# kausaltech/reina-model

Measured on NVIDIA B200. Metric: agent-days/sec (HUS 1.7M), higher is better.
Workload: dtype int32/f32 state, f64 uniforms

## Files before the change

### reina_b200/csrc/engine.cu

```cuda
#include "state.cuh"
#include "boundary.cuh"
#include "sweep.cuh"
#include "contacts.cuh"
#include "shard.cuh"
#include "setup.cuh"
#include "run.cuh"

static thread_local char g_err[512];
#define CK(call) do { cudaError_t e_ = (call); if (e_ != cudaSuccess) { snprintf(g_err, sizeof g_err, "%s:%d %s: %s", __FILE__, __LINE__, #call, cudaGetErrorString(e_)); return 1; } } while (0)

#define MAX_GROUPS 8
struct ReplicaGroup {
    int r0, R;
    int sweep_blocks, list_blocks, resolve_blocks;
    cudaStream_t stream;
    cudaEvent_t ev_stagger, ev_join;
    cudaGraphExec_t graph[2];
};

struct rb_engine {
    rb_config cfg;
    Eng G;
    cudaStream_t stream;
    cudaEvent_t ev0, ev1;
// ... 47 lines not shown
static int load_nccl() {
    if (g_nccl.dl) return 0;
    void *h = dlopen("libnccl.so.2", RTLD_NOW | RTLD_NOLOAD | RTLD_GLOBAL);
    if (!h) h = dlopen("libnccl.so.2", RTLD_NOW | RTLD_GLOBAL);
    if (!h) h = dlopen("libnccl.so", RTLD_NOW | RTLD_GLOBAL);
    if (!h) { snprintf(g_err, sizeof g_err, "cannot load libnccl.so.2: %s", dlerror()); return 1; }
    g_nccl.GetUniqueId = (ncclResult_t(*)(ncclUniqueId *))dlsym(h, "ncclGetUniqueId");
    g_nccl.CommInitRank = (ncclResult_t(*)(ncclComm_t *, int, ncclUniqueId, int))dlsym(h, "ncclCommInitRank");
    g_nccl.AllGather = (ncclResult_t(*)(const void *, void *, size_t, ncclDataType_t, ncclComm_t, cudaStream_t))dlsym(h, "ncclAllGather");
    g_nccl.AllReduce = (ncclResult_t(*)(const void *, void *, size_t, ncclDataType_t, ncclRedOp_t, ncclComm_t, cudaStream_t))dlsym(h, "ncclAllReduce");
    g_nccl.CommDestroy = (ncclResult_t(*)(ncclComm_t))dlsym(h, "ncclCommDestroy");
    g_nccl.GetErrorString = (const char *(*)(ncclResult_t))dlsym(h, "ncclGetErrorString");
    if (!g_nccl.GetUniqueId || !g_nccl.CommInitRank || !g_nccl.AllGather || !g_nccl.AllReduce || !g_nccl.CommDestroy || !g_nccl.GetErrorString) {
        snprintf(g_err, sizeof g_err, "libnccl.so.2 lacks a required symbol"); return 1;
    }
    g_nccl.dl = h;
    return 0;
}
#define NK(call) do { ncclResult_t r_ = (call); if (r_ != ncclSuccess) { snprintf(g_err, sizeof g_err, "%s:%d %s: %s", __FILE__, __LINE__, #call, g_nccl.GetErrorString(r_)); return 1; } } while (0)


template <typename T> static int dalloc(rb_engine *e, T **p, size_t n) {
    void *q = nullptr;
    cudaError_t err = cudaMalloc(&q, n * sizeof(T));
    if (err != cudaSuccess) { snprintf(g_err, sizeof g_err, "cudaMalloc(%zu bytes): %s", n * sizeof(T), cudaGetErrorString(err)); return 1; }
    e->allocs.push_back(q);
    *p = (T *)q;
    return 0;
}
static uint32_t pow2_at_least(uint64_t x) { uint32_t p = 1024; while (p < x) p <<= 1; return p; }

extern "C" const char *rb_last_error(void) { return g_err; }

static int init_population(rb_engine *e, uint32_t seed, bool sparse) {
    const Eng &G = e->G;
    k_init_counters<<<G.R, 128, 0, e->stream>>>(G, seed, e->cfg.hospital_beds, e->cfg.icu_units);
    if (sparse) k_init<true><<<dim3(e->sweep_blocks, G.R), 256, 0, e->stream>>>(G);
    else k_init<false><<<dim3(e->sweep_blocks, G.R), 256, 0, e->stream>>>(G);
    k_init_bitmaps<<<dim3(8, G.R), 256, 0, e->stream>>>(G);
    k_clear_lists<<<128, 256, 0, e->stream>>>(G);
    e->launches += 4;
    CK(cudaGetLastError());
    return 0;
}

static int setup_groups(rb_engine *e, int sms);
static void group_config(int R, int *n_groups, int *wave_pct);

static int resolve_grid(int n_agents, int sms, int pct, int replicas) {
    long long b = ((long long)n_agents / 128 + 255) / 256;
    long long cap = (long long)sms * 16 * pct / 100 / replicas; if (cap < 64) cap = 64;
    if (const char *s = getenv("RB_RESOLVE_BLOCKS")) cap = b = atoi(s);
    if (b > cap) b = cap;
    return b < 1 ? 1 : (int)b;
}

extern "C" void rb_destroy(rb_engine *e) {
    if (!e) return;
    cudaSetDevice(e->cfg.device);
    cudaStreamSynchronize(e->stream);
    if (e->have_graphs) {
        if (e->n_groups <= 1) { cudaGraphExecDestroy(e->graph[0]); cudaGraphExecDestroy(e->graph[1]); }
        else for (int g = 0; g < e->n_groups; g++) { cudaGraphExecDestroy(e->grp[g].graph[0]); cudaGraphExecDestroy(e->grp[g].graph[1]); }
    }
    for (int g = 0; g < e->n_groups && e->n_groups > 1; g++) {
        cudaStreamDestroy(e->grp[g].stream); cudaEventDestroy(e->grp[g].ev_stagger); cudaEventDestroy(e->grp[g].ev_join);
    }
    if (e->n_groups > 1) cudaEventDestroy(e->ev_fork);
    if (e->have_sh_graphs) { cudaGraphExecDestroy(e->sh_graph[0]); cudaGraphExecDestroy(e->sh_graph[1]); }
    for (int k = 0; k < e->n_peer_open; k++) if (k != e->G.rank && e->G.xpeer[k]) cudaIpcCloseMemHandle(e->G.xpeer[k]);
    if (e->comm) g_nccl.CommDestroy(e->comm);
    for (void *p : e->allocs) cudaFree(p);
    if (e->h_stage) { cudaFreeHost(e->h_stage); for (int i = 0; i < 4; i++) cudaEventDestroy(e->ev_stage[i]); }
    cudaEventDestroy(e->ev0); cudaEventDestroy(e->ev1);
    cudaStreamDestroy(e->stream);
    delete e;
}

extern "C" int rb_create(const rb_config *cfg, const int32_t *age_counts, const int32_t *group_of_age,
                         const rb_variant *variants, const int32_t *import_lo, const int32_t *import_hi,
                         const float *import_cum, rb_engine **out) {
    if (cfg->n_ages > RB_MAX_AGES || cfg->n_variants > RB_MAX_VARIANTS || cfg->n_import_classes > RB_MAX_IMPORT_CLASSES ||
        cfg->n_groups > 16 || cfg->n_replicas < 1 || cfg->n_agents < 1) {
        snprintf(g_err, sizeof g_err, "config exceeds compiled limits"); return 1;
    }
    int ndev = 0;
    if (cudaGetDeviceCount(&ndev) != cudaSuccess || ndev == 0) {
        snprintf(g_err, sizeof g_err, "no CUDA device: reina_b200 has no CPU fallback"); return 2;
    }
    CK(cudaSetDevice(cfg->device));
    if (const char *s = getenv("RB_L2_FETCH")) cudaDeviceSetLimit(cudaLimitMaxL2FetchGranularity, (size_t)atoi(s));
    rb_engine *e = new rb_engine();
    e->cfg = *cfg; e->day = 0; e->last_ms = 0; e->launches = 0; e->h2d_bytes = 0; e->d2h_bytes = 0; e->have_graphs = false; e->comm = nullptr; e->comm_rank = 0; e->comm_size = 1; e->sharded = false; e->merge_blocks = 1;
    e->has_ipc = false; e->h_stage = nullptr; e->n_stage = 0; e->n_groups = 1; e->wide_ctas = 1; e->n_peer_open = 0; e->launch_err = cudaSuccess; e->shard_timing = getenv("RB_SHARD_TIMING") != nullptr;
    e->xepoch = 0; e->d_xepoch = nullptr; e->have_sh_graphs = false;
    { int lo = 0, hi = 0; CK(cudaDeviceGetStreamPriorityRange(&lo, &hi)); e->prio_high = hi; e->prio = (cfg->n_replicas >= 32 && cfg->n_replicas < 128) ? 1 : 0; if (const char *s = getenv("RB_PRIO")) e->prio = atoi(s); }
    CK(cudaStreamCreateWithFlags(&e->stream, cudaStreamNonBlocking));
    CK(cudaEventCreate(&e->ev0)); CK(cudaEventCreate(&e->ev1));
    Eng &G = e->G;
    memset(&G, 0, sizeof G);
    const int N = cfg->n_agents, R = cfg->n_replicas;
    G.N = N; G.Npad = (N + 3) & ~3; G.n_ages = cfg->n_ages; G.n_groups = cfg->n_groups; G.n_variants = cfg->n_variants;
    G.R = R; G.max_days = cfg->max_days; G.row_len = RB_N_ATTRS * cfg->n_groups + RB_N_SCALARS;
    G.n_import_classes = cfg->n_import_classes;
    G.rank = 0; G.nranks = 1;
    int bits = 1; while ((1u << bits) < (uint32_t)N) bits++;
    G.fhalf = (bits + 1) / 2;
    e->age_start.resize(cfg->n_ages + 1);
    int64_t tot = 0;
    for (int a = 0; a < cfg->n_ages; a++) { e->age_start[a] = (int32_t)tot; tot += age_counts[a]; }
    e->age_start[cfg->n_ages] = (int32_t)tot;
    if (tot != N) { snprintf(g_err, sizeof g_err, "age_counts sum %lld != n_agents %d", (long long)tot, N); delete e; return 1; }
    for (int i = 0; i < cfg->n_import_classes; i++) {
        const float w = import_cum[i] - (i ? import_cum[i - 1] : 0.0f);
        if (import_lo[i] < 0 || import_hi[i] >= cfg->n_ages || import_lo[i] > import_hi[i]) { snprintf(g_err, sizeof g_err, "import class %d: bad age band", i); delete e; return 1; }
        if ((w > 0.0f || i == cfg->n_import_classes - 1) && e->age_start[import_hi[i] + 1] - e->age_start[import_lo[i]] <= 0) {
            snprintf(g_err, sizeof g_err, "import class %d (ages %d-%d) can be drawn but is empty", i, import_lo[i], import_hi[i]); delete e; return 1;
        }
    }
    float cc = cfg->contact_capacity > 0 ? cfg->contact_capacity : 1.0f;
    G.cap_items = pow2_at_least((uint64_t)((double)N * cc) + 4096);
    G.cap_succ = pow2_at_least((uint64_t)N / 8 + 4096);
    G.cap_events = pow2_at_least((uint64_t)N / 16 + 2048);
    G.cap_queue = pow2_at_least((uint64_t)N / 8 + 2048);
    const size_t RN = (size_t)R * G.Npad;
    cudaDeviceProp prop; CK(cudaGetDeviceProperties(&prop, cfg->device));
    const int sms = prop.multiProcessorCount;
    e->run_ctas = 0; e->run_boundary_ctas = 1;
    {
        int per_sm = 0;
        CK(cudaOccupancyMaxActiveBlocksPerMultiprocessor(&per_sm, k_run, RUN_THREADS, 0));
        const long long total = (long long)per_sm * sms;
        bool on = false;
        if (const char *s = getenv("RB_PERSISTENT")) on = atoi(s) != 0;
        if (on && total >= 2LL * R) {
            long long t = total / R; if (t > 64) t = 64;
            if (const char *s = getenv("RB_RUN_CTAS")) { const int v = atoi(s); if (v >= 1 && (long long)v * R <= total) t = v; }
            e->run_ctas = (int)t;
            int b = 1; while (b * 2 <= t && b * 2 <= 16) b *= 2;
            e->run_boundary_ctas = b;
        }
    }
    {
        int ng, pct;
        group_config(R, &ng, &pct);
        long long ctas = (long long)sms * SW_CTAS_PER_SM * (ng > 1 ? pct : 100) / 100 / ((R + ng - 1) / ng);
        if (ctas < 1) ctas = 1;
        long long S = 2 * ctas * SW_WARPS, most = (long long)N / 256;
        if (e->run_ctas) S = 2LL * e->run_ctas * RUN_WARPS;
        if (S > most) S = most;
        G.n_seg = (uint32_t)(S < 1 ? 1 : S);
        G.seg_cap = ((uint32_t)N + G.n_seg - 1) / G.n_seg;
    }
    G.sus_words = ((G.Npad + 31) / 32 + 32 + 3) & ~3;
    if (dalloc(e, &G.hot, RN) || dalloc(e, &G.perm, RN) || dalloc(e, &G.rec, RN) ||
        dalloc(e, &G.sus, (size_t)R * G.sus_words) || dalloc(e, &G.det, (size_t)R * G.sus_words) || dalloc(e, &G.alist, (size_t)R * 2 * G.n_seg * G.seg_cap) || dalloc(e, &G.seg_n, (size_t)R * 2 * G.n_seg) || dalloc(e, &G.items, (size_t)R * G.cap_items) || dalloc(e, &G.succ, (size_t)R * G.cap_succ) ||
        dalloc(e, &G.ev_key, (size_t)R * G.cap_events) || dalloc(e, &G.ev_agent, (size_t)R * G.cap_events) ||
        dalloc(e, &G.q_key, (size_t)R * 2 * G.cap_queue) || dalloc(e, &G.q_agent, (size_t)R * 2 * G.cap_queue) ||
        dalloc(e, &G.ctr, (size_t)R) || dalloc(e, &G.stats, (size_t)R * (cfg->max_days + 1) * G.row_len) ||
        dalloc(e, &e->d_sched, (size_t)cfg->max_days + 1) ||
        dalloc(e, &e->d_moments, 2 * ((size_t)cfg->max_days + 1) * G.row_len + 2)) { rb_destroy(e); return 1; }
    G.sched = e->d_sched;
    e->h_sched.assign(cfg->max_days + 1, rb_day_params());
    e->n_table_slots = 1024;
    if (dalloc(e, &e->d_tables, (size_t)e->n_table_slots)) { rb_destroy(e); return 1; }
    CK(cudaMemset(e->d_tables, 0, sizeof(DevTable *) * e->n_table_slots));
    G.tables = e->d_tables;
    e->tables.assign(e->n_table_slots, nullptr);
    rb_variant *dv; int32_t *d_as, *d_ga, *d_ilo, *d_ihi; float *d_icum; uint8_t *d_ab;
    if (dalloc(e, &dv, (size_t)cfg->n_variants) || dalloc(e, &d_as, (size_t)cfg->n_ages + 1) || dalloc(e, &d_ga, (size_t)cfg->n_ages) ||
        dalloc(e, &d_ilo, (size_t)RB_MAX_IMPORT_CLASSES) || dalloc(e, &d_ihi, (size_t)RB_MAX_IMPORT_CLASSES) ||
        dalloc(e, &d_icum, (size_t)RB_MAX_IMPORT_CLASSES) || dalloc(e, &d_ab, (size_t)(G.Npad >> 10) + 2)) { rb_destroy(e); return 1; }
    {
        std::vector<uint8_t> ab((size_t)(G.Npad >> 10) + 2);
        int age = 0;
        for (size_t b = 0; b < ab.size(); b++) {
            int64_t a = (int64_t)b << 10; if (a > N - 1) a = N - 1;
            while (age < cfg->n_ages - 1 && e->age_start[age + 1] <= a) age++;
            ab[b] = (uint8_t)age;
        }
        CK(cudaMemcpy(d_ab, ab.data(), ab.size(), cudaMemcpyHostToDevice));
    }
    e->h_variants.assign(variants, variants + cfg->n_variants);
    CK(cudaMemcpy(dv, variants, sizeof(rb_variant) * cfg->n_variants, cudaMemcpyHostToDevice));
    CK(cudaMemcpy(d_as, e->age_start.data(), sizeof(int32_t) * (cfg->n_ages + 1), cudaMemcpyHostToDevice));
    CK(cudaMemcpy(d_ga, group_of_age, sizeof(int32_t) * cfg->n_ages, cudaMemcpyHostToDevice));
    CK(cudaMemcpy(d_ilo, import_lo, sizeof(int32_t) * cfg->n_import_classes, cudaMemcpyHostToDevice));
    CK(cudaMemcpy(d_ihi, import_hi, sizeof(int32_t) * cfg->n_import_classes, cudaMemcpyHostToDevice));
    CK(cudaMemcpy(d_icum, import_cum, sizeof(float) * cfg->n_import_classes, cudaMemcpyHostToDevice));
    G.age_blk = d_ab; G.variants = dv; G.age_start = d_as; G.group_of_age = d_ga; G.import_lo = d_ilo; G.import_hi = d_ihi; G.import_cum = d_icum;
    e->age_counts.assign(age_counts, age_counts + cfg->n_ages);
    CK(cudaMemset(G.stats, 0, sizeof(int32_t) * (size_t)R * (cfg->max_days + 1) * G.row_len));
    CK(cudaMemset(e->d_sched, 0, sizeof(rb_day_params) * ((size_t)cfg->max_days + 1)));
    int want = ((int)G.n_seg + SW_WARPS - 1) / SW_WARPS;
    int per_rep = sms * SW_CTAS_PER_SM / R; if (per_rep < 1) per_rep = 1;
    e->sweep_blocks = want < per_rep ? want : per_rep; if (e->sweep_blocks < 1) e->sweep_blocks = 1;
    e->list_blocks = sms * EX_CTAS_PER_SM / R; if (e->list_blocks < 2) e->list_blocks = 2;
    e->resolve_blocks = resolve_grid(G.N, sms, 100, R);
    if (init_population(e, cfg->seed, false)) { rb_destroy(e); return 1; }
    CK(cudaStreamSynchronize(e->stream));
    if (e->run_ctas) e->n_groups = 1;
    else if (setup_groups(e, sms)) { rb_destroy(e); return 1; }
    e->wide_ctas = 1;
    G.wide_min = 2048;
    if (e->n_groups == 1 && R * 4 <= sms && N >= 4000000) { e->wide_ctas = 16; while (e->wide_ctas * R > sms) e->wide_ctas >>= 1; }
    if (const char *s = getenv("RB_WIDE_CTAS")) { int v = atoi(s); if (v >= 1 && v <= WIDE_MAX_CTAS && v * R <= sms) e->wide_ctas = v; }
    if (const char *s = getenv("RB_WIDE_MIN")) G.wide_min = atoi(s);
    if (const char *s = getenv("RB_WIDE_CTAS")) {
        const int v = atoi(s); int b = 1; while (b * 2 <= v && b * 2 <= e->run_ctas) b *= 2;
        if (e->run_ctas) e->run_boundary_ctas = b;
    }
    *out = e;
    return 0;
}

static void group_config(int R, int *n_groups, int *wave_pct) {
    int ng = R >= 32 ? 4 : 1, pct = R >= 32 ? 50 : 100;
    if (const char *s = getenv("RB_GROUPS")) ng = atoi(s);
    if (const char *s = getenv("RB_GROUP_WAVE_PCT")) pct = atoi(s);
    if (pct < 1) pct = 100;
    if (ng > MAX_GROUPS) ng = MAX_GROUPS;
    if (ng > R) ng = R;
    if (ng < 1) ng = 1;
    *n_groups = ng; *wave_pct = pct;
}
static int setup_groups(rb_engine *e, int sms) {
    const int R = e->G.R;
    int ng, pct;
    group_config(R, &ng, &pct);
    e->n_groups = ng;
    if (ng == 1) return 0;
    CK(cudaEventCreateWithFlags(&e->ev_fork, cudaEventDisableTiming));
    const Eng &G = e->G;
    const int want = ((int)G.n_seg + SW_WARPS - 1) / SW_WARPS;
    for (int g = 0; g < ng; g++) {
        ReplicaGroup &q = e->grp[g];
        q.r0 = (int)((long long)R * g / ng); q.R = (int)((long long)R * (g + 1) / ng) - q.r0;
        int per = sms * SW_CTAS_PER_SM * pct / 100 / q.R; if (per < 1) per = 1;
        q.sweep_blocks = want < per ? want : per;
        q.list_blocks = sms * EX_CTAS_PER_SM * pct / 100 / q.R; if (q.list_blocks < 2) q.list_blocks = 2;
        q.resolve_blocks = resolve_grid(G.N, sms, pct, q.R);
        CK(cudaStreamCreateWithFlags(&q.stream, cudaStreamNonBlocking));
        CK(cudaEventCreateWithFlags(&q.ev_stagger, cudaEventDisableTiming));
        CK(cudaEventCreateWithFlags(&q.ev_join, cudaEventDisableTiming));
    }
    return 0;
}

__global__ void k_set_word(uint32_t *p, uint32_t v) { *p = v; }
static void bump_xepoch(rb_engine *e) {
    e->xepoch++;
    if (e->d_xepoch) { k_set_word<<<1, 1, 0, e->stream>>>(e->d_xepoch, e->xepoch); e->launches++; }
}

extern "C" int rb_reset(rb_engine *e, uint32_t seed) {
    CK(cudaSetDevice(e->cfg.device));
    CK(cudaStreamSynchronize(e->stream));
    e->cfg.seed = seed;
    e->day = 0;
    bump_xepoch(e);
    if (init_population(e, seed, true)) return 1;
    if (e->has_ipc) {
        k_initial_state<<<e->G.R, 32, 0, e->stream>>>(e->G, e->ipc);
        k_rebuild_lists<<<dim3(e->sweep_blocks, e->G.R), 256, 0, e->stream>>>(e->G);
        e->launches += 2;
    }
    CK(cudaGetLastError());
    return 0;
}

extern "C" int rb_set_initial_state(rb_engine *e, const int32_t *ipc7) {
    CK(cudaSetDevice(e->cfg.device));
    if (e->day != 0 || e->has_ipc) { snprintf(g_err, sizeof g_err, "rb_set_initial_state: once, before the first step"); return 1; }
    for (int i = 0; i < 7; i++) if (ipc7[i] < 0) { snprintf(g_err, sizeof g_err, "rb_set_initial_state: negative count"); return 1; }
    e->ipc.dead = ipc7[0]; e->ipc.in_icu = ipc7[1]; e->ipc.in_ward = ipc7[2]; e->ipc.confirmed = ipc7[3];
    e->ipc.incubating = ipc7[4]; e->ipc.ill = ipc7[5]; e->ipc.recovered = ipc7[6];
    e->has_ipc = true;
    k_initial_state<<<e->G.R, 32, 0, e->stream>>>(e->G, e->ipc);
    k_rebuild_lists<<<dim3(e->sweep_blocks, e->G.R), 256, 0, e->stream>>>(e->G);
    e->launches += 2;
    CK(cudaGetLastError());
    CK(cudaStreamSynchronize(e->stream));
    return 0;
}

#define TABLE_HOST_BYTES (offsetof(DevTable, guide))
static int stage_slot(rb_engine *e, DevTable **h, int *slot) {
    if (!e->h_stage) {
        CK(cudaMallocHost((void **)&e->h_stage, TABLE_HOST_BYTES * 4));
        for (int i = 0; i < 4; i++) CK(cudaEventCreateWithFlags(&e->ev_stage[i], cudaEventDisableTiming));
        e->n_stage = 0;
    }
    const int k = e->n_stage & 3;
    if (e->n_stage >= 4) CK(cudaEventSynchronize(e->ev_stage[k]));
    e->n_stage++;
    *h = (DevTable *)((uint8_t *)e->h_stage + TABLE_HOST_BYTES * k); *slot = k;
    return 0;
}

extern "C" int rb_set_contact_table(rb_engine *e, int32_t epoch, const int32_t *n_rows, const double *cum_p,
                                    const int32_t *age_lo, const int32_t *age_hi, const uint8_t *place,
                                    const float *mask_p, const double *nr_contacts, const double *ncontact_cdf) {
    if (epoch < 0 || epoch >= e->n_table_slots) { snprintf(g_err, sizeof g_err, "table epoch out of range"); return 1; }
    CK(cudaSetDevice(e->cfg.device));
    for (int age = 0; age < e->cfg.n_ages; age++) {
        if (n_rows[age] < 0 || n_rows[age] > RB_MAX_ROWS) { snprintf(g_err, sizeof g_err, "contact table: n_rows[%d] = %d", age, n_rows[age]); return 1; }
        if (e->age_counts[age] == 0) continue;
        for (int i = 0; i < n_rows[age]; i++) {
            const int k = age * RB_MAX_ROWS + i;
// ... 804 lines not shown
```

### reina_b200/csrc/state.cuh

```cuda
#ifndef REINA_B200_STATE_CUH
#define REINA_B200_STATE_CUH

#include <cuda_runtime.h>
#include <stdint.h>
#include <stdio.h>
#include <string.h>

#include <dlfcn.h>
#include <nccl.h>

#include <algorithm>
#include <vector>

#include "../../include/reina_b200.h"
#include "rng.cuh"

#define MAX_INFECTEES 64
#define MAX_CONTACTS 128

#define H_STATE(h) ((h) & 7u)
#define H_SEV(h) (((h) >> 3) & 7u)
#define H_DET (1u << 6)
#define H_QUEUED (1u << 7)
#define H_VAR(h) (((h) >> 8) & 3u)
#define H_FRESH (1u << 10)
#define H_INCL (1u << 11)
#define H_LIST (1u << 12)
#define H_VACC (1u << 13)
#define H_DL(h) (((h) >> 14) & 255u)
#define H_DOI(h) (((h) >> 22) & 31u)
#define H_PEND (1u << 27)
#define H_DAYS_MASK ((255u << 14) | (31u << 22))
#define H_SET_STATE(h, s) (((h) & ~7u) | (uint32_t)(s))
#define H_SET_DL(h, d) (((h) & ~(255u << 14)) | ((uint32_t)(d) << 14))
#define H_SET_DOI(h, d) (((h) & ~(31u << 22)) | ((uint32_t)(d) << 22))

#define KEY_IDLE 0xFFFFFFFFFFFFFFFFull
#define QKEY_SWEEP (1ull << 62)
#define CT_DEAD (1ull << 61)
#define CT_DECIDED (1ull << 60)
#define CT_KEYMASK ((1ull << 60) - 1ull)

enum { EV_HOSP_CLAIM = 0, EV_WARD_RELEASE = 1, EV_TO_ICU = 2, EV_ICU_RELEASE = 3 };

#define MAX_RANKS 16
#define WIDE_MAX_CTAS 64
#define SORT_SMEM 2048
#ifndef PRE_THREADS
#define PRE_THREADS 512
#endif
#define NEG_INF (-(1 << 29))

#ifndef GUIDE_BITS
#define GUIDE_BITS 12
#endif
struct DevTable {
    int32_t n_rows[RB_MAX_AGES];
    float nr_contacts[RB_MAX_AGES];
    double ncdf[RB_MAX_AGES][2][RB_NCDF];
    double cum_p[RB_MAX_AGES][RB_MAX_ROWS];
    uint32_t cum24[RB_MAX_AGES][RB_MAX_ROWS];
    int32_t start[RB_MAX_AGES][RB_MAX_ROWS];
    int32_t size[RB_MAX_AGES][RB_MAX_ROWS];
    float mask_p[RB_MAX_AGES][RB_MAX_ROWS];
    uint8_t place[RB_MAX_AGES][RB_MAX_ROWS];
    uint8_t lo_age[RB_MAX_AGES][RB_MAX_ROWS], hi_age[RB_MAX_AGES][RB_MAX_ROWS];
    uint8_t susc_uniform[RB_MAX_AGES][RB_MAX_ROWS];
    uint8_t nguide[RB_MAX_AGES][2][256];
    uint32_t guide[RB_MAX_AGES][1 << GUIDE_BITS];
};

struct Attempt { uint32_t cand, parent; unsigned long long key; };

struct __align__(32) AgentRec {
    unsigned long long winner;
    int32_t infector, first_child, next_sib;
    uint32_t inf_key;
    uint32_t cold;
    int16_t vacc_day, pad;
};

struct RepCtr {
    int32_t counts[RB_N_ATTRS][RB_MAX_AGES];
    alignas(128) int32_t beds;
    int32_t icu, avail_beds, avail_icu;
    int32_t problem, epoch, testing_mode, day;
    float p_detected_anyway, p_successful_tracing;
    uint32_t seed, start;
    uint32_t fkey[4];
    uint32_t n_queue, qsel;
    uint32_t n_queue_prev;
    uint32_t any_vacc;
    uint32_t lsel;
    uint32_t ct_ever;
    uint32_t n_q_base;
    uint32_t drained;
    int32_t ct_cases;
    int32_t vacc_cursor[RB_MAX_VACC];
    alignas(128) uint32_t n_items;
    alignas(128) uint32_t n_succ;
    alignas(128) int32_t exposed_per_day;
    int32_t total_infectors, total_infections;
    alignas(128) uint32_t n_events;
    uint32_t n_newq;
    uint32_t n_upd;
    alignas(128) int32_t daily_contacts[RB_N_PLACES];
    int32_t by_variant[RB_MAX_VARIANTS];
    alignas(128) int32_t drain_det[RB_MAX_AGES];
    alignas(128) uint32_t n_l0;
    uint32_t n_l1, n_edges;
    alignas(128) unsigned int run_bar;
    unsigned int run_exit;
    alignas(128) unsigned int wide_bar;
    alignas(128) uint32_t wide_day;
    int32_t wide_mp[WIDE_MAX_CTAS][4];
    long long dbg_t[16];
    long long dbg_last;
};

struct Eng {
    int32_t dbg;
    int32_t N, Npad, n_ages, n_groups, n_variants, R, max_days, row_len, n_import_classes, fhalf;
    uint32_t cap_items, cap_succ, cap_events, cap_queue;
    uint32_t *hot;
    uint32_t *perm;
    AgentRec *rec;
    uint32_t *sus;
    int32_t sus_words;
    uint32_t *det;
    uint2 *alist;
    uint2 *seg_n;
    uint32_t n_seg, seg_cap;
    uint2 *items;
    Attempt *succ;
    unsigned long long *ev_key; int32_t *ev_agent;
    unsigned long long *q_key; int32_t *q_agent;
    RepCtr *ctr;
    int32_t *stats;
    const rb_day_params *sched;
    DevTable *const *tables;
    const rb_variant *variants;
    const int32_t *age_start;
    const uint8_t *age_blk;
    const int32_t *group_of_age;
    const int32_t *import_lo, *import_hi; const float *import_cum;
    int32_t rank, nranks;
    int32_t wide_min;
    int32_t r0;
    uint8_t *xbuf; size_t xslot;
    uint8_t *xpeer[MAX_RANKS];
    int32_t xp2p; const uint32_t *xepoch;
    uint32_t xcap_q, xcap_ev, xcap_upd, xcap_succ;
};

#define XFLAG_BYTES 256
#define SH_SHIFT 12
__device__ __forceinline__ uint32_t xflag_value(const Eng &G, int day) { return *G.xepoch * 65536u + (uint32_t)day + 1u; }
__device__ __forceinline__ bool owns(const Eng &G, uint32_t a) { return G.nranks == 1 || (int)((a >> SH_SHIFT) % (uint32_t)G.nranks) == G.rank; }

struct XSlot {
    RepCtr *hdr;
    unsigned long long *q_key; int32_t *q_agent;
    unsigned long long *ev_key; int32_t *ev_agent;
    uint2 *upd;
    struct Attempt *succ;
};
__host__ __device__ inline size_t xalign(size_t x) { return (x + 255) & ~(size_t)255; }
__host__ __device__ inline size_t xslot_bytes(uint32_t cq, uint32_t ce, uint32_t cu, uint32_t cs) {
    return xalign(sizeof(RepCtr)) + xalign(8ull * cq) + xalign(4ull * cq) + xalign(8ull * ce) + xalign(4ull * ce) + xalign(8ull * cu) + xalign(16ull * cs);
}
__device__ __forceinline__ XSlot xslot_of(const Eng &G, int rk, int day) {
    uint8_t *p = G.xp2p ? G.xpeer[rk] + XFLAG_BYTES + (size_t)(day & 1) * G.xslot : G.xbuf + (size_t)rk * G.xslot;
    XSlot s;
    s.hdr = (RepCtr *)p; p += xalign(sizeof(RepCtr));
    s.q_key = (unsigned long long *)p; p += xalign(8ull * G.xcap_q);
    s.q_agent = (int32_t *)p; p += xalign(4ull * G.xcap_q);
    s.ev_key = (unsigned long long *)p; p += xalign(8ull * G.xcap_ev);
    s.ev_agent = (int32_t *)p; p += xalign(4ull * G.xcap_ev);
    s.upd = (uint2 *)p; p += xalign(8ull * G.xcap_upd);
    s.succ = (struct Attempt *)p;
    return s;
}

__device__ __forceinline__ int age_of(const Eng &G, int32_t a) {
    int age = __ldg(&G.age_blk[a >> 10]);
    while (a >= __ldg(&G.age_start[age + 1])) age++;
    return age;
}
__device__ __forceinline__ int age_in_band(const Eng &G, int32_t a, int lo, int hi) {
    hi += 1;
    while (hi - lo > 1) { int mid = (lo + hi) >> 1; if (__ldg(&G.age_start[mid]) <= a) lo = mid; else hi = mid; }
    return lo;
}
__device__ __forceinline__ uint32_t sweep_slot(const Eng &G, const RepCtr *c, uint32_t a) {
    return feistel(a, (uint32_t)G.N, G.fhalf, c->fkey[0], c->fkey[1], c->fkey[2], c->fkey[3]);
}
__device__ __forceinline__ uint32_t sweep_pos(const Eng &G, int r, const RepCtr *c, uint32_t a) {
    const uint32_t s = G.perm[(size_t)r * G.Npad + a];
    return s >= c->start ? s - c->start : s + (uint32_t)G.N - c->start;
}
__device__ __forceinline__ void mark_detected(const Eng &G, int r, int32_t a) {
    atomicOr(&G.det[(size_t)r * G.sus_words + (a >> 5)], 1u << (a & 31));
}
__device__ __forceinline__ void count_add(RepCtr *c, int attr, int age, int d) { atomicAdd(&c->counts[attr][age], d); }
__device__ __forceinline__ void set_problem(RepCtr *c, int p) { atomicCAS(&c->problem, 0, p); }

__device__ __forceinline__ int symptom_severity(const rb_variant *v, int age, float val, bool vacc_eff) {
    float vmod = 1.0f;
    if (vacc_eff) vmod = vmod * 0.1f;
    float syc = v->tab[RB_T_SYMPTOMATIC][age];
    if (val >= syc) return RB_ASYMPTOMATIC;
    syc = syc * vmod;
    float dohc = v->tab[RB_T_DEATH_OUTSIDE_HOSPITAL][age];
    if (dohc != 0.0f) {
        if (val < dohc * syc) return RB_FATAL;
        val = (val - dohc) / (1.0f - dohc);
    }
    float sc = v->tab[RB_T_SEVERE][age], cc = v->tab[RB_T_CRITICAL][age], fc = v->tab[RB_T_FATAL][age];
    if (val < ((fc * cc) * sc) * syc) return RB_FATAL;
    if (val < (cc * sc) * syc) return RB_CRITICAL;
    if (val < sc * syc) return RB_SEVERE;
    return RB_MILD;
}

__device__ __forceinline__ uint2 *seg_ptr(const Eng &G, int r, uint32_t which, uint32_t s) {
    return G.alist + (((size_t)r * 2 + which) * G.n_seg + s) * G.seg_cap;
}
__device__ __forceinline__ uint2 *seg_count(const Eng &G, int r, uint32_t which, uint32_t s) {
    return G.seg_n + ((size_t)r * 2 + which) * G.n_seg + s;
}
__device__ __forceinline__ void list_add(const Eng &G, int r, RepCtr *c, uint32_t which, uint32_t a, uint32_t w) {
    const uint32_t s = a % G.n_seg;
    const uint32_t k = atomicAdd(&seg_count(G, r, which, s)->y, 1u);
    if (k < G.seg_cap) seg_ptr(G, r, which, s)[G.seg_cap - 1u - k] = make_uint2(a, w); else set_problem(c, RB_OTHER_FAILURE);
}

__device__ void device_infect(const Eng &G, int r, RepCtr *c, int32_t t, int32_t src, uint32_t src_h, int variant,
                              int slot, bool fresh, int list, bool has_list) {
    const size_t base = (size_t)r * G.Npad;
    const int day = c->day;
    uint32_t old = 0; int32_t prev_child = -1;
    if (src >= 0) {
        old = atomicAdd(&G.rec[base + src].cold, 1u);
        prev_child = atomicExch(&G.rec[base + src].first_child, t);
    }
    const int vd = c->any_vacc ? (int)G.rec[base + t].vacc_day : -1;
    const int age = age_of(G, t);
    const rb_variant *v0 = &G.variants[0];
    const bool vacc_eff = vd >= 0 && (day - vd) > 14;
    int sev = 0, dl = 0;
    if (owns(G, (uint32_t)t)) {
        u32x4 x = philox(c->seed, (uint32_t)t, (uint32_t)day, PU_SEVERITY, 0);
        sev = symptom_severity(v0, age, u01f(x.x), vacc_eff);
        dl = clamp255(round_to_int(gamma_f(c->seed, (uint32_t)t, (uint32_t)day, PU_INCUB, v0->incubation_kappa, v0->incubation_theta)));
    }
    if (src >= 0) {
        variant = (int)H_VAR(src_h);
        G.rec[base + t].infector = src;
        if ((src_h & H_LIST) && (old & 0xffffu) >= MAX_INFECTEES) set_problem(c, RB_TOO_MANY_INFECTEES);
        G.rec[base + t].inf_key = ((uint32_t)day << 8) | (uint32_t)slot;
        G.rec[base + t].next_sib = prev_child;
    }
    uint32_t nh = (vd >= 0 ? H_VACC : 0u) | RB_INCUBATION | ((uint32_t)sev << 3) | ((uint32_t)variant << 8) | ((uint32_t)dl << 14);
    if (fresh) nh |= H_FRESH;
    if (has_list) nh |= H_LIST;
    G.hot[base + t] = nh;
    G.perm[base + t] = sweep_slot(G, c, (uint32_t)t);
    atomicAnd(&G.sus[(size_t)r * G.sus_words + (t >> 5)], ~(1u << (t & 31)));
    if (list >= 0 && owns(G, (uint32_t)t)) list_add(G, r, c, (uint32_t)list, (uint32_t)t, nh);
    count_add(c, RB_A_SUSCEPTIBLE, age, -1);
    count_add(c, RB_A_INFECTED, age, 1);
    count_add(c, RB_A_ALL_INFECTED, age, 1);
    count_add(c, RB_A_NEW_INFECTIONS, age, 1);
    {
        const unsigned act = __activemask();
        const unsigned grp = __match_any_sync(act, variant);
        if ((int)(threadIdx.x & 31) == __ffs(grp) - 1) atomicAdd(&c->by_variant[variant], __popc(grp));
    }
}

#endif
```

### reina_b200/csrc/sweep.cuh

```cuda
#ifndef REINA_B200_SWEEP_CUH
#define REINA_B200_SWEEP_CUH
#include "state.cuh"

#ifndef SW_THREADS
#define SW_THREADS 128
#endif
#define SW_WARPS (SW_THREADS / 32)
#define SW_RCAP 64
#ifndef SW_CTAS_PER_SM
#define SW_CTAS_PER_SM 9
#endif

struct WarpRings {
    uint32_t ea[SW_RCAP], ed[SW_RCAP];
    uint32_t ta[SW_RCAP], tw[SW_RCAP];
};

__device__ __forceinline__ uint32_t ring_push(uint32_t *ra, uint32_t *rb, uint32_t tail, bool want, uint32_t x, uint32_t y, int lane) {
    const uint32_t m = __ballot_sync(0xffffffffu, want);
    if (want) { uint32_t p = (tail + __popc(m & ((1u << lane) - 1u))) & (SW_RCAP - 1); ra[p] = x; rb[p] = y; }
    return tail + __popc(m);
}

__device__ __forceinline__ void seg_append(const Eng &G, RepCtr *c, uint2 *out, uint32_t &out_n, bool want, uint32_t a, uint32_t w, int lane) {
    const uint32_t m = __ballot_sync(0xffffffffu, want);
    if (want) {
        const uint32_t p = out_n + __popc(m & ((1u << lane) - 1u));
        if (p < G.seg_cap) out[p] = make_uint2(a, w); else set_problem(c, RB_OTHER_FAILURE);
    }
    out_n += __popc(m);
}

struct SweepOut {
    RepCtr *cd;
    unsigned long long *q_key; int32_t *q_agent; uint32_t cap_q;
    unsigned long long *ev_key; int32_t *ev_agent; uint32_t cap_ev;
    uint2 *upd; uint32_t cap_upd;
};
__device__ __forceinline__ SweepOut sweep_out(const Eng &G, int r, RepCtr *c) {
    SweepOut O;
    if (!G.xbuf) {
        const size_t qb = ((size_t)r * 2 + (c->qsel ^ 1u)) * G.cap_queue;
        O.cd = c; O.q_key = G.q_key + qb; O.q_agent = G.q_agent + qb; O.cap_q = G.cap_queue;
        O.ev_key = G.ev_key + (size_t)r * G.cap_events; O.ev_agent = G.ev_agent + (size_t)r * G.cap_events; O.cap_ev = G.cap_events;
        O.upd = nullptr; O.cap_upd = 0;
    } else {
        const XSlot x = xslot_of(G, G.rank, c->day);
        O.cd = x.hdr; O.q_key = x.q_key; O.q_agent = x.q_agent; O.cap_q = G.xcap_q;
        O.ev_key = x.ev_key; O.ev_agent = x.ev_agent; O.cap_ev = G.xcap_ev; O.upd = x.upd; O.cap_upd = G.xcap_upd;
    }
    return O;
}

__device__ __forceinline__ void stage_expose(const Eng &G, int r, RepCtr *c, RepCtr *cd, const DevTable *tb, const WarpRings &W, uint32_t head, uint32_t m,
                                             uint2 *items, int lane) {
    uint32_t ncont = 0, desc = 0, a = 0;
    if ((uint32_t)lane < m) {
        a = W.ea[(head + lane) & (SW_RCAP - 1)];
        desc = W.ed[(head + lane) & (SW_RCAP - 1)];
        bool detected = false;
        if (c->ct_ever) detected = (__ldg(&G.det[(size_t)r * G.sus_words + (a >> 5)]) >> (a & 31)) & 1u;
        if (!detected) {
            const int age = age_of(G, (int32_t)a);
            const int cls = (desc >> 22) & 1u;
            u32x4 x = philox(c->seed, a, (uint32_t)c->day, PU_NCONTACT, 0);
            const double u = u01d(x.x, x.y);
            const double *cdf = tb->ncdf[age][cls];
            const int limit = cls ? 5 : 100;
            const uint32_t ng = tb->nguide[age][cls][x.x >> 24];
            int k = (int)(ng & 127u);
            if (ng & 128u) while (k < limit && !(u < __ldg(&cdf[k]))) k++;
            ncont = (uint32_t)k;
            desc = (desc & ~(1u << 22)) | ((uint32_t)age << 7);
        }
    }
    const uint32_t cnt = (ncont + 3u) >> 2;
    uint32_t incl = cnt | (ncont << 16);
#pragma unroll
    for (int o = 1; o < 32; o <<= 1) { uint32_t t = __shfl_up_sync(0xffffffffu, incl, o); if (lane >= o) incl += t; }
    const uint32_t tot = __shfl_sync(0xffffffffu, incl, 31), wtot = tot & 0xffffu;
    if (wtot == 0) return;
    uint32_t gbase = 0;
    if (lane == 31) { gbase = atomicAdd(&c->n_items, wtot); atomicAdd(&cd->exposed_per_day, (int)(tot >> 16)); }
    gbase = __shfl_sync(0xffffffffu, gbase, 31);
    if (gbase + wtot > G.cap_items) { if (lane == 0) set_problem(cd, RB_OTHER_FAILURE); return; }
    uint2 *mine = items + gbase + ((incl & 0xffffu) - cnt);
    for (uint32_t g = 0; g < cnt; g++) {
        const uint32_t left = ncont - 4u * g;
        mine[g] = make_uint2(a, desc | g | (((left < 4u ? left : 4u) - 1u) << 5));
    }
}

__device__ __forceinline__ void emit_event(const Eng &G, int r, const SweepOut &O, RepCtr *c, int32_t a, int type) {
    uint32_t idx = atomicAdd(&O.cd->n_events, 1u);
    if (idx < O.cap_ev) {
        O.ev_key[idx] = ((unsigned long long)sweep_pos(G, r, c, (uint32_t)a) << 2) | (unsigned)type;
        O.ev_agent[idx] = a;
    } else set_problem(O.cd, RB_OTHER_FAILURE);
}

__device__ __forceinline__ uint32_t transition(const Eng &G, int r, RepCtr *c, const SweepOut &O, int32_t a, uint32_t h, uint32_t &lw) {
    RepCtr *cd = O.cd;
    const size_t base = (size_t)r * G.Npad;
    const int day = c->day;
    const int age = age_of(G, a);
    const uint32_t st = H_STATE(h), sev = H_SEV(h);
    const rb_variant *v = &G.variants[H_VAR(h)];
    uint32_t extra = 0;
    if (st == RB_INCUBATION) {
        float T = (sev == RB_FATAL)
            ? gamma_f(c->seed, (uint32_t)a, (uint32_t)day, PU_ONSET, v->onset_death_kappa, v->onset_death_theta)
            : gamma_f(c->seed, (uint32_t)a, (uint32_t)day, PU_ONSET, v->onset_recovery_kappa, v->onset_recovery_theta);
        float f = T;
        if (sev != RB_ASYMPTOMATIC && sev != RB_MILD) f = f * v->ratio_before_hospitalisation;
        const uint32_t dl = (uint32_t)clamp255(round_to_int(f));
        float w = 0.0f, u = 0.0f;
        if (sev == RB_SEVERE) w = T * (1.0f - v->ratio_before_hospitalisation);
        else if (sev == RB_CRITICAL || sev == RB_FATAL) {
            w = T * v->ratio_in_ward;
            u = ((1.0f - v->ratio_in_ward) - v->ratio_before_hospitalisation) * T;
        }
        const uint32_t wd = (uint32_t)clamp255(round_to_int(w)), ud = (uint32_t)clamp255(round_to_int(u));
        if (wd | ud) atomicOr(&G.rec[base + a].cold, (wd << 16) | (ud << 24));
        h = H_SET_DL(H_SET_STATE(h, RB_ILLNESS), dl);
        if (sev != RB_ASYMPTOMATIC && !(h & H_DET)) {
            bool q = false;
            const int mode = c->testing_mode;
            if (mode == RB_ALL_WITH_SYMPTOMS || mode == RB_ALL_WITH_SYMPTOMS_CT) q = true;
            else if (mode == RB_ONLY_SEVERE_SYMPTOMS) {
                if (sev >= RB_SEVERE) q = true;
                else {
                    u32x4 x = philox(c->seed, (uint32_t)a, (uint32_t)day, PU_SEEK, 0);
                    q = chance(u01d(x.x, x.y), c->p_detected_anyway);
                }
            }
            if (q && !(h & H_QUEUED)) {
                h |= H_QUEUED;
                uint32_t idx = atomicAdd(&cd->n_newq, 1u);
                if (idx < O.cap_q) {
                    O.q_key[idx] = QKEY_SWEEP | sweep_pos(G, r, c, (uint32_t)a);
                    O.q_agent[idx] = a;
                } else set_problem(cd, RB_OTHER_FAILURE);
            }
        }
        if (h & H_QUEUED) extra = H_DET;
    } else if (st == RB_ILLNESS) {
        if (sev == RB_FATAL) {
            h = H_SET_STATE(h, RB_DEAD) & ~H_LIST;
            count_add(cd, RB_A_INFECTED, age, -1); count_add(cd, RB_A_DEAD, age, 1); count_add(cd, RB_A_NON_HOSPITAL_DEATHS, age, 1);
        } else if (sev >= RB_SEVERE) {
            if (!(h & H_DET)) { h |= H_DET; count_add(cd, RB_A_DETECTED, age, 1); count_add(cd, RB_A_ALL_DETECTED, age, 1); }
            emit_event(G, r, O, c, a, EV_HOSP_CLAIM);
            extra = H_PEND;
        } else {
            h = H_SET_STATE(h, RB_RECOVERED) & ~H_LIST;
            count_add(cd, RB_A_INFECTED, age, -1); count_add(cd, RB_A_RECOVERED, age, 1);
        }
    } else {
        int type;
        if (st == RB_HOSPITALIZED && (sev == RB_CRITICAL || sev == RB_FATAL)) { type = EV_TO_ICU; extra = H_PEND; }
        else {
            type = st == RB_IN_ICU ? EV_ICU_RELEASE : EV_WARD_RELEASE;
            count_add(cd, st == RB_IN_ICU ? RB_A_IN_ICU : RB_A_IN_WARD, age, -1);
            count_add(cd, RB_A_INFECTED, age, -1);
            if (sev == RB_FATAL) { h = H_SET_STATE(h, RB_DEAD) & ~H_LIST; count_add(cd, RB_A_DEAD, age, 1); count_add(cd, RB_A_NON_HOSPITAL_DEATHS, age, 1); }
            else { h = H_SET_STATE(h, RB_RECOVERED) & ~H_LIST; count_add(cd, RB_A_RECOVERED, age, 1); }
        }
        emit_event(G, r, O, c, a, type);
    }
    lw = h | extra;
    return h;
}

__device__ __forceinline__ void stage_slow(const Eng &G, int r, RepCtr *c, RepCtr *cd, const WarpRings &W, uint32_t head, uint32_t m,
                                           uint32_t next, int lane) {
    const SweepOut O = sweep_out(G, r, c);
    const size_t base = (size_t)r * G.Npad;
    const bool on = (uint32_t)lane < m;
    bool keep = false, changed = false, removed = false;
    int infected_others = 0;
    uint32_t a = 0, lw = 0, h = 0;
    if (on) {
        a = W.ta[(head + lane) & (SW_RCAP - 1)];
        const uint32_t w = W.tw[(head + lane) & (SW_RCAP - 1)];
        const uint32_t hot = G.hot[base + a];
        if (w & H_PEND) {
            h = hot & ~H_FRESH;
            if (H_STATE(h) < RB_RECOVERED) { uint32_t dl = H_DL(h); if (dl > 0) dl--; h = H_SET_DL(h, dl); }
        } else h = (hot & ~(H_DAYS_MASK | H_FRESH)) | (w & H_DAYS_MASK);
        const uint32_t st = H_STATE(h);
        if (st >= RB_RECOVERED) {
            removed = true;
            infected_others = (int)(G.rec[base + a].cold & 0xffffu);
            G.hot[base + a] = hot | H_INCL;
        } else if (H_DL(h) == 0) {
            h = transition(G, r, c, O, (int32_t)a, h, lw);
            G.hot[base + a] = h;
            keep = true; changed = true;
        } else { lw = h; keep = true; }
    }
    const uint32_t rm = __ballot_sync(0xffffffffu, removed);
    if (rm) {
#pragma unroll
        for (int o = 16; o > 0; o >>= 1) infected_others += __shfl_xor_sync(0xffffffffu, infected_others, o);
        if (lane == 0) { atomicAdd(&cd->total_infectors, __popc(rm)); if (infected_others) atomicAdd(&cd->total_infections, infected_others); }
    }
    if (keep) list_add(G, r, cd, next, a, lw);
    if (O.upd) {
        const uint32_t mk = __ballot_sync(0xffffffffu, changed);
        uint32_t b = 0;
        if (lane == 0 && mk) b = atomicAdd(&O.cd->n_upd, (uint32_t)__popc(mk));
        b = __shfl_sync(0xffffffffu, b, 0);
        if (changed) {
            const uint32_t idx = b + __popc(mk & ((1u << lane) - 1u));
            if (idx < O.cap_upd) O.upd[idx] = make_uint2(a, h); else set_problem(O.cd, RB_OTHER_FAILURE);
        }
    }
}

__device__ __forceinline__ void stage_entry(const Eng &G, uint32_t &w, bool &keep, bool &want_e, bool &want_t, uint32_t &desc) {
    const uint32_t st = H_STATE(w);
    if ((w & H_PEND) || st >= RB_RECOVERED) { want_t = true; return; }
    if (w & H_FRESH) { w &= ~H_FRESH; keep = true; return; }
    const uint32_t sev = H_SEV(w), var = H_VAR(w);
    uint32_t dl = H_DL(w);
    if (st == RB_INCUBATION || st == RB_ILLNESS) {
        const int dayidx = st == RB_INCUBATION ? -(int)dl : (int)H_DOI(w);
        if (!(w & H_DET) && dayidx >= -10 && dayidx <= 10 && G.variants[var].iot[dayidx + 10] != 0.0f) {
            want_e = true;
            const uint32_t cls = (st == RB_ILLNESS && sev != RB_ASYMPTOMATIC) ? 1u : 0u;
            desc = ((uint32_t)(dayidx + 10) << 14) | ((sev == RB_ASYMPTOMATIC ? 1u : 0u) << 19) | (var << 20) | (cls << 22);
        }
        if (st == RB_ILLNESS) { uint32_t doi = H_DOI(w); if (doi < 31) doi++; w = H_SET_DOI(w, doi); }
    }
    if (dl > 0) dl--;
    w = H_SET_DL(w, dl);
    if (dl == 0) want_t = true; else keep = true;
}

__device__ __forceinline__ void sweep_warp(const Eng &G, const int r, const uint32_t first, const uint32_t n_warps, WarpRings &W, const int lane) {
    RepCtr *c = &G.ctr[r];
    const DevTable *tb = G.tables[c->epoch];
    uint2 *items = G.items + (size_t)r * G.cap_items;
    RepCtr *cd = !G.xbuf ? c : xslot_of(G, G.rank, c->day).hdr;
    const uint32_t cur = c->lsel;
    uint32_t e_head = 0, e_tail = 0, t_head = 0, t_tail = 0;

    uint2 cnt_next = make_uint2(0u, 0u);
    if (first < G.n_seg) cnt_next = *seg_count(G, r, cur, first);
    for (uint32_t seg = first; ; seg += n_warps) {
        const bool tail = seg >= G.n_seg;
        const uint2 cnt = cnt_next;
        cnt_next = make_uint2(0u, 0u);
        if (seg + n_warps < G.n_seg) cnt_next = *seg_count(G, r, cur, seg + n_warps);
        const uint32_t nf = min(cnt.x, G.seg_cap), n = min(cnt.x + cnt.y, G.seg_cap);
        const uint2 *in = seg_ptr(G, r, cur, tail ? 0u : seg);
        uint2 *out = seg_ptr(G, r, cur ^ 1u, tail ? 0u : seg);
        uint32_t out_n = 0;
        const uint32_t gap = G.seg_cap - n;
        auto entry = [&](uint32_t i) { return __ldcs(&in[i < nf ? i : i + gap]); };
        uint2 ent = make_uint2(0u, 0u);
        if ((uint32_t)lane < n) ent = entry(lane);
        uint32_t i0 = 0;
        bool again;
        do {
            if (i0 < n) {
                const bool valid = i0 + lane < n;
                const uint2 cur_ent = ent;
                if (i0 + 32 + lane < n) ent = entry(i0 + 32 + lane);
                bool keep = false, want_e = false, want_t = false;
                uint32_t w = cur_ent.y, desc = 0;
                if (valid) stage_entry(G, w, keep, want_e, want_t, desc);
                seg_append(G, cd, out, out_n, keep, cur_ent.x, w, lane);
                e_tail = ring_push(W.ea, W.ed, e_tail, want_e, cur_ent.x, desc, lane);
                t_tail = ring_push(W.ta, W.tw, t_tail, want_t, cur_ent.x, w, lane);
                __syncwarp();
            }
            const uint32_t e_av = e_tail - e_head, t_av = t_tail - t_head;
            if (e_av >= 32 || (tail && e_av)) { const uint32_t m = min(32u, e_av); stage_expose(G, r, c, cd, tb, W, e_head, m, items, lane); e_head += m; }
            if (t_av >= 32 || (tail && t_av)) { const uint32_t m = min(32u, t_av); stage_slow(G, r, c, cd, W, t_head, m, cur ^ 1u, lane); t_head += m; }
            __syncwarp();
            i0 += 32;
            again = tail ? (e_tail != e_head || t_tail != t_head) : i0 < n;
        } while (again);
        if (tail) break;
        if (lane == 0) seg_count(G, r, cur ^ 1u, seg)->x = out_n;
    }
}
__global__ void __launch_bounds__(SW_THREADS, SW_CTAS_PER_SM) k_sweep(Eng G) {
    __shared__ WarpRings s_rings[SW_WARPS];
    const int warp = threadIdx.x >> 5;
    sweep_warp(G, blockIdx.y + G.r0, blockIdx.x * SW_WARPS + warp, gridDim.x * SW_WARPS, s_rings[warp], threadIdx.x & 31);
}

__global__ void k_flush_lists(Eng G) {
    const int r = blockIdx.y;
    const RepCtr *c = &G.ctr[r];
    const size_t base = (size_t)r * G.Npad;
    const uint32_t cur = c->lsel;
    const int lane = threadIdx.x & 31;
    const uint32_t n_warps = gridDim.x * (blockDim.x >> 5);
    for (uint32_t seg = blockIdx.x * (blockDim.x >> 5) + (threadIdx.x >> 5); seg < G.n_seg; seg += n_warps) {
        const uint2 cnt = *seg_count(G, r, cur, seg);
        const uint32_t nf = min(cnt.x, G.seg_cap), n = min(cnt.x + cnt.y, G.seg_cap);
        const uint2 *in = seg_ptr(G, r, cur, seg);
        for (uint32_t i = lane; i < n; i += 32) {
            const uint2 e = in[i < nf ? i : i + (G.seg_cap - n)];
            if ((e.y & H_PEND) || H_STATE(e.y) >= RB_RECOVERED) continue;
            const uint32_t h = G.hot[base + e.x];
            G.hot[base + e.x] = (h & ~(H_DAYS_MASK | H_FRESH)) | (e.y & (H_DAYS_MASK | H_FRESH));
        }
    }
}
__global__ void k_rebuild_lists(Eng G) {
    const int r = blockIdx.y;
    RepCtr *c = &G.ctr[r];
    const size_t base = (size_t)r * G.Npad;
    const uint32_t cur = c->lsel;
    for (int a = blockIdx.x * blockDim.x + threadIdx.x; a < G.N; a += gridDim.x * blockDim.x) {
        if (!owns(G, (uint32_t)a)) continue;
        uint32_t h = G.hot[base + a];
        const uint32_t st = H_STATE(h);
        if (!((st >= RB_INCUBATION && st <= RB_IN_ICU) || (st >= RB_RECOVERED && !(h & H_INCL)))) continue;
        if (h & H_QUEUED) h |= H_DET;
        G.perm[base + a] = sweep_slot(G, c, (uint32_t)a);
        list_add(G, r, c, cur, (uint32_t)a, h);
    }
}
__global__ void k_clear_lists(Eng G) {
    const size_t n = (size_t)G.R * 2 * G.n_seg;
    for (size_t i = (size_t)blockIdx.x * blockDim.x + threadIdx.x; i < n; i += (size_t)gridDim.x * blockDim.x) G.seg_n[i] = make_uint2(0u, 0u);
}

#endif
```

Before: 744.4 billion.

## Park idle agents in a per-segment timing wheel to skip daily sweeps

Adds a 32-slot timing wheel per segment. Agents whose next state change lies several days away are parked into the slot for their wake-up day instead of being rewritten to the active list each day. When the wheel slot comes due, parked agents are merged back into the sweep with their day counters advanced in bulk. Flushing and clearing are extended to cover parked entries. The aim is to cut per-day read, classify and write traffic for agents with nothing to do. The cost is extra memory, warp match/ballot work per batch, and a risk of losing entries if a wheel slot overflows its capacity.

```diff
diff --git a/reina_b200/csrc/engine.cu b/reina_b200/csrc/engine.cu
--- a/reina_b200/csrc/engine.cu
+++ b/reina_b200/csrc/engine.cu
@@ -223,9 +223,17 @@
         G.n_seg = (uint32_t)(S < 1 ? 1 : S);
         G.seg_cap = ((uint32_t)N + G.n_seg - 1) / G.n_seg;
     }
+    G.wheel_cap = G.seg_cap / 16 + 8;
+    if (const char *s = getenv("RB_WHEEL_CAP")) G.wheel_cap = (uint32_t)atoi(s);
+    for (int v = 0; v < cfg->n_variants; v++) {
+        G.park_inc[v] = 0; G.park_ill[v] = 0;
+        for (int x = 1; x <= 10; x++) if (variants[v].iot[10 - x] != 0.0f) G.park_inc[v] |= 1u << x;
+        for (int x = 0; x <= 10; x++) if (variants[v].iot[10 + x] != 0.0f) G.park_ill[v] |= 1u << x;
+    }
     G.sus_words = ((G.Npad + 31) / 32 + 32 + 3) & ~3;
     if (dalloc(e, &G.hot, RN) || dalloc(e, &G.perm, RN) || dalloc(e, &G.rec, RN) ||
-        dalloc(e, &G.sus, (size_t)R * G.sus_words) || dalloc(e, &G.det, (size_t)R * G.sus_words) || dalloc(e, &G.alist, (size_t)R * 2 * G.n_seg * G.seg_cap) || dalloc(e, &G.seg_n, (size_t)R * 2 * G.n_seg) || dalloc(e, &G.items, (size_t)R * G.cap_items) || dalloc(e, &G.succ, (size_t)R * G.cap_succ) ||
+        dalloc(e, &G.sus, (size_t)R * G.sus_words) || dalloc(e, &G.det, (size_t)R * G.sus_words) || dalloc(e, &G.alist, (size_t)R * 2 * G.n_seg * G.seg_cap) || dalloc(e, &G.seg_n, (size_t)R * 2 * G.n_seg) ||
+        dalloc(e, &G.wheel, (size_t)R * G.n_seg * WHEEL_W * G.wheel_cap) || dalloc(e, &G.wheel_n, (size_t)R * G.n_seg * WHEEL_W) || dalloc(e, &G.items, (size_t)R * G.cap_items) || dalloc(e, &G.succ, (size_t)R * G.cap_succ) ||
         dalloc(e, &G.ev_key, (size_t)R * G.cap_events) || dalloc(e, &G.ev_agent, (size_t)R * G.cap_events) ||
         dalloc(e, &G.q_key, (size_t)R * 2 * G.cap_queue) || dalloc(e, &G.q_agent, (size_t)R * 2 * G.cap_queue) ||
         dalloc(e, &G.ctr, (size_t)R) || dalloc(e, &G.stats, (size_t)R * (cfg->max_days + 1) * G.row_len) ||
diff --git a/reina_b200/csrc/state.cuh b/reina_b200/csrc/state.cuh
--- a/reina_b200/csrc/state.cuh
+++ b/reina_b200/csrc/state.cuh
@@ -131,6 +131,11 @@
     uint2 *alist;
     uint2 *seg_n;
     uint32_t n_seg, seg_cap;
+    uint2 *wheel;
+    uint32_t *wheel_n;
+    uint32_t wheel_cap;
+    uint32_t park_inc[RB_MAX_VARIANTS];
+    uint32_t park_ill[RB_MAX_VARIANTS];
     uint2 *items;
     Attempt *succ;
     unsigned long long *ev_key; int32_t *ev_agent;
@@ -229,6 +234,12 @@
 __device__ __forceinline__ uint2 *seg_count(const Eng &G, int r, uint32_t which, uint32_t s) {
     return G.seg_n + ((size_t)r * 2 + which) * G.n_seg + s;
 }
+#define WHEEL_W 32
+#define WH_K_SHIFT 27
+__device__ __forceinline__ uint2 *wheel_ptr(const Eng &G, int r, uint32_t s, uint32_t b) {
+    return G.wheel + (((size_t)r * G.n_seg + s) * WHEEL_W + b) * G.wheel_cap;
+}
+__device__ __forceinline__ uint32_t *wheel_count(const Eng &G, int r, uint32_t s) { return G.wheel_n + ((size_t)r * G.n_seg + s) * WHEEL_W; }
 __device__ __forceinline__ void list_add(const Eng &G, int r, RepCtr *c, uint32_t which, uint32_t a, uint32_t w) {
     const uint32_t s = a % G.n_seg;
     const uint32_t k = atomicAdd(&seg_count(G, r, which, s)->y, 1u);
diff --git a/reina_b200/csrc/sweep.cuh b/reina_b200/csrc/sweep.cuh
--- a/reina_b200/csrc/sweep.cuh
+++ b/reina_b200/csrc/sweep.cuh
@@ -7,6 +7,9 @@
 #endif
 #define SW_WARPS (SW_THREADS / 32)
 #define SW_RCAP 64
+#ifndef PARK_MIN_K
+#define PARK_MIN_K 2
+#endif
 #ifndef SW_CTAS_PER_SM
 #define SW_CTAS_PER_SM 9
 #endif
@@ -14,6 +17,7 @@
 struct WarpRings {
     uint32_t ea[SW_RCAP], ed[SW_RCAP];
     uint32_t ta[SW_RCAP], tw[SW_RCAP];
+    uint32_t wn[WHEEL_W];
 };
 
 __device__ __forceinline__ uint32_t ring_push(uint32_t *ra, uint32_t *rb, uint32_t tail, bool want, uint32_t x, uint32_t y, int lane) {
@@ -238,6 +242,44 @@
     if (dl == 0) want_t = true; else keep = true;
 }
 
+__device__ __forceinline__ uint32_t count_down(uint32_t w, uint32_t j) {
+    w = H_SET_DL(w, H_DL(w) - j);
+    if (H_STATE(w) == RB_ILLNESS) w = H_SET_DOI(w, min(31u, H_DOI(w) + j));
+    return w;
+}
+__device__ __forceinline__ uint32_t wake_word(uint32_t ws) { return count_down(ws & ((1u << WH_K_SHIFT) - 1u), ws >> WH_K_SHIFT); }
+__device__ __forceinline__ uint32_t park_days(const Eng &G, uint32_t w) {
+    const uint32_t dl = H_DL(w), st = H_STATE(w);
+    if (dl < 3) return 0;
+    uint32_t k = dl - 1;
+    if (!(w & H_DET)) {
+        if (st == RB_INCUBATION) {
+            const uint32_t m = G.park_inc[H_VAR(w)] & (dl >= 31 ? ~0u : (2u << dl) - 1u);
+            if (m) k = min(k, dl - (31u - (uint32_t)__clz(m)));
+        } else if (st == RB_ILLNESS) {
+            const uint32_t doi = H_DOI(w), m = G.park_ill[H_VAR(w)] & (~0u << doi);
+            if (m) k = min(k, (uint32_t)(__ffs(m) - 1) - doi);
+        }
+    }
+    k = min(k, (uint32_t)WHEEL_W - 2u);
+    return k >= PARK_MIN_K ? k : 0u;
+}
+__device__ __forceinline__ bool park(const Eng &G, int r, uint32_t seg, uint32_t day, WarpRings &W, bool keep, uint32_t a, uint32_t w, int lane) {
+    const uint32_t k = keep ? park_days(G, w) : 0u;
+    if (!__any_sync(0xffffffffu, k != 0u)) return false;
+    const uint32_t b = k ? (day + k + 1u) % WHEEL_W : WHEEL_W;
+    const uint32_t grp = __match_any_sync(0xffffffffu, b);
+    const uint32_t base = k ? W.wn[b] : 0u;
+    __syncwarp();
+    if (k && lane == __ffs(grp) - 1) W.wn[b] = base + __popc(grp);
+    __syncwarp();
+    if (!k) return false;
+    const uint32_t idx = base + __popc(grp & ((1u << lane) - 1u));
+    if (idx >= G.wheel_cap) return false;
+    wheel_ptr(G, r, seg, b)[idx] = make_uint2(a, w | (k << WH_K_SHIFT));
+    return true;
+}
+
 __device__ __forceinline__ void sweep_warp(const Eng &G, const int r, const uint32_t first, const uint32_t n_warps, WarpRings &W, const int lane) {
     RepCtr *c = &G.ctr[r];
     const DevTable *tb = G.tables[c->epoch];
@@ -247,30 +289,39 @@
     uint32_t e_head = 0, e_tail = 0, t_head = 0, t_tail = 0;
 
     uint2 cnt_next = make_uint2(0u, 0u);
-    if (first < G.n_seg) cnt_next = *seg_count(G, r, cur, first);
+    uint32_t wn_next = 0;
+    if (first < G.n_seg) { cnt_next = *seg_count(G, r, cur, first); wn_next = wheel_count(G, r, first)[lane]; }
     for (uint32_t seg = first; ; seg += n_warps) {
         const bool tail = seg >= G.n_seg;
         const uint2 cnt = cnt_next;
+        const uint32_t wn = wn_next;
+        W.wn[lane] = wn;
+        __syncwarp();
         cnt_next = make_uint2(0u, 0u);
-        if (seg + n_warps < G.n_seg) cnt_next = *seg_count(G, r, cur, seg + n_warps);
+        wn_next = 0;
+        if (seg + n_warps < G.n_seg) { cnt_next = *seg_count(G, r, cur, seg + n_warps); wn_next = wheel_count(G, r, seg + n_warps)[lane]; }
         const uint32_t nf = min(cnt.x, G.seg_cap), n = min(cnt.x + cnt.y, G.seg_cap);
+        const uint32_t today = (uint32_t)c->day % WHEEL_W;
+        const uint32_t nt = n + min(__shfl_sync(0xffffffffu, wn, today), G.wheel_cap);
         const uint2 *in = seg_ptr(G, r, cur, tail ? 0u : seg);
+        const uint2 *wk = wheel_ptr(G, r, tail ? 0u : seg, today);
         uint2 *out = seg_ptr(G, r, cur ^ 1u, tail ? 0u : seg);
         uint32_t out_n = 0;
         const uint32_t gap = G.seg_cap - n;
-        auto entry = [&](uint32_t i) { return __ldcs(&in[i < nf ? i : i + gap]); };
+        auto entry = [&](uint32_t i) { return __ldcs(i < nf ? &in[i] : (i < n ? &in[i + gap] : &wk[i - n])); };
         uint2 ent = make_uint2(0u, 0u);
-        if ((uint32_t)lane < n) ent = entry(lane);
+        if ((uint32_t)lane < nt) ent = entry(lane);
         uint32_t i0 = 0;
         bool again;
         do {
-            if (i0 < n) {
-                const bool valid = i0 + lane < n;
+            if (i0 < nt) {
+                const bool valid = i0 + lane < nt;
                 const uint2 cur_ent = ent;
-                if (i0 + 32 + lane < n) ent = entry(i0 + 32 + lane);
+                if (i0 + 32 + lane < nt) ent = entry(i0 + 32 + lane);
                 bool keep = false, want_e = false, want_t = false;
-                uint32_t w = cur_ent.y, desc = 0;
+                uint32_t w = i0 + lane >= n ? wake_word(cur_ent.y) : cur_ent.y, desc = 0;
                 if (valid) stage_entry(G, w, keep, want_e, want_t, desc);
+                if (park(G, r, seg, (uint32_t)c->day, W, keep, cur_ent.x, w, lane)) keep = false;
                 seg_append(G, cd, out, out_n, keep, cur_ent.x, w, lane);
                 e_tail = ring_push(W.ea, W.ed, e_tail, want_e, cur_ent.x, desc, lane);
                 t_tail = ring_push(W.ta, W.tw, t_tail, want_t, cur_ent.x, w, lane);
@@ -281,10 +332,12 @@
             if (t_av >= 32 || (tail && t_av)) { const uint32_t m = min(32u, t_av); stage_slow(G, r, c, cd, W, t_head, m, cur ^ 1u, lane); t_head += m; }
             __syncwarp();
             i0 += 32;
-            again = tail ? (e_tail != e_head || t_tail != t_head) : i0 < n;
+            again = tail ? (e_tail != e_head || t_tail != t_head) : i0 < nt;
         } while (again);
         if (tail) break;
         if (lane == 0) seg_count(G, r, cur ^ 1u, seg)->x = out_n;
+        wheel_count(G, r, seg)[lane] = lane == (int)today ? 0u : W.wn[lane];
+        __syncwarp();
     }
 }
 __global__ void __launch_bounds__(SW_THREADS, SW_CTAS_PER_SM) k_sweep(Eng G) {
@@ -311,6 +364,19 @@
             G.hot[base + e.x] = (h & ~(H_DAYS_MASK | H_FRESH)) | (e.y & (H_DAYS_MASK | H_FRESH));
         }
     }
+    const uint32_t day = (uint32_t)c->day;
+    for (uint32_t seg = blockIdx.x * (blockDim.x >> 5) + (threadIdx.x >> 5); seg < G.n_seg; seg += n_warps) {
+        for (uint32_t b = 0; b < WHEEL_W; b++) {
+            const uint32_t n = min(wheel_count(G, r, seg)[b], G.wheel_cap), ahead = (b + WHEEL_W - day % WHEEL_W) % WHEEL_W;
+            const uint2 *in = wheel_ptr(G, r, seg, b);
+            for (uint32_t i = lane; i < n; i += 32) {
+                const uint2 e = in[i];
+                const uint32_t w = count_down(e.y & ((1u << WH_K_SHIFT) - 1u), (e.y >> WH_K_SHIFT) - ahead);
+                const uint32_t h = G.hot[base + e.x];
+                G.hot[base + e.x] = (h & ~(H_DAYS_MASK | H_FRESH)) | (w & H_DAYS_MASK);
+            }
+        }
+    }
 }
 __global__ void k_rebuild_lists(Eng G) {
     const int r = blockIdx.y;
@@ -330,6 +396,7 @@
 __global__ void k_clear_lists(Eng G) {
     const size_t n = (size_t)G.R * 2 * G.n_seg;
     for (size_t i = (size_t)blockIdx.x * blockDim.x + threadIdx.x; i < n; i += (size_t)gridDim.x * blockDim.x) G.seg_n[i] = make_uint2(0u, 0u);
+    for (size_t i = (size_t)blockIdx.x * blockDim.x + threadIdx.x; i < (size_t)G.R * G.n_seg * WHEEL_W; i += (size_t)gridDim.x * blockDim.x) G.wheel_n[i] = 0u;
 }
 
 #endif
```

Result: faster. 765.6 billion (median of 6 runs) (+2.8%).
